# Napoliee/Expressive-FastSpeech2-Mandarin

Measured on AMD Instinct MI355X. Metric: mel-frames/sec/GPU (batch-64 synth) at 1/2/4/8 MI355X; RTF, higher is better.
Workload: dtype bf16; 1 GPU; cfg2: batch=64 x 64 phonemes per GPU, ESD-Chinese-Singing-MFA model.yaml, FastSpeech2.forward eval bf16; global_batch=64, seq_len=64, mel_frames_per_gpu_batch=24883, T_max=430, parallelism=dp1 (independent shards, no collective), hip_graph=True

## Files before the change

expressive-fastspeech2-mandarin_amd/csrc/lr.hip:

```cpp
#include <cstdlib>
#include <type_traits>

#include "fs2_common.h"
#include "fs2hip_prosody.h"

namespace {

constexpr int kScanThreads = 256;
constexpr int kLdsCum = 2048;

__device__ __forceinline__ int64_t frames_of(const void *dur, int kind, float d_control, const float *d_map,
                                             int64_t idx, float *d_rounded) {
  if (kind == FS2_DUR_I64) {
    int64_t d = reinterpret_cast<const int64_t *>(dur)[idx];
    return d > 0 ? d : 0;
  }
  float v = reinterpret_cast<const float *>(dur)[idx];
  if (kind == FS2_DUR_LOGPRED) {
    float r = rintf(expf(v) - 1.0f) * (d_map != nullptr ? d_map[idx] : d_control);
    r = r < 0.0f ? 0.0f : r;
    if (d_rounded) d_rounded[idx] = r;
    v = r;
  }
  if (!(v > 0.0f)) return 0;
  if (v >= 9.2e18f) return INT64_MAX / 4;
  return (int64_t)v;
}

__global__ __launch_bounds__(kScanThreads) void lr_durations_kernel(const void *dur, int kind, float d_control,
                                                                    const float *d_map, int L, int32_t *cum,
                                                                    int64_t *mel_len, float *d_rounded) {
  const int b = blockIdx.x;
  const int tid = threadIdx.x;
  const int lane = tid & 63, wid = tid >> 6;
  const int per = (L + kScanThreads - 1) / kScanThreads;
  const int i0 = min(tid * per, L), i1 = min(i0 + per, L);
  const int64_t base = (int64_t)b * L;
// ... 330 lines not shown
    bf16 *pb = a.proj_out + ((int64_t)cu_b + t0) * NP;
    const int lanes = 192 / cg * cg;
    if (tid < lanes) {
      const int c = (tid % cg) * 8, r1 = tid / cg, rs = lanes / cg;
      for (int r0 = r1; r0 < rows; r0 += RB * rs) {
        float4 tv[RB][2], sv[RB][2];
#pragma unroll
        for (int u = 0; u < RB; ++u) {
          const int r = min(r0 + u * rs, rows - 1);
          const int sidx = src[r];
          const float *tp = tb + (int64_t)r * NP + c;
          tv[u][0] = *reinterpret_cast<const float4 *>(tp);
          tv[u][1] = *reinterpret_cast<const float4 *>(tp + 4);
          if (sidx >= 0) {
            const float *sp = sb + (int64_t)sidx * NP + c;
            sv[u][0] = *reinterpret_cast<const float4 *>(sp);
            sv[u][1] = *reinterpret_cast<const float4 *>(sp + 4);
          } else {
            sv[u][0] = sv[u][1] = make_float4(0.f, 0.f, 0.f, 0.f);
          }
        }
#pragma unroll
        for (int u = 0; u < RB; ++u) {
          const int r = r0 + u * rs;
          if (r < rows) {
            const bf16x8 o{(bf16)(tv[u][0].x + sv[u][0].x), (bf16)(tv[u][0].y + sv[u][0].y),
                           (bf16)(tv[u][0].z + sv[u][0].z), (bf16)(tv[u][0].w + sv[u][0].w),
                           (bf16)(tv[u][1].x + sv[u][1].x), (bf16)(tv[u][1].y + sv[u][1].y),
                           (bf16)(tv[u][1].z + sv[u][1].z), (bf16)(tv[u][1].w + sv[u][1].w)};
            __builtin_nontemporal_store(o, reinterpret_cast<bf16x8 *>(pb + (int64_t)r * NP + c));
          }
        }
      }
    }
  }
}

__global__ __launch_bounds__(256) void length_mask_kernel(const int64_t *__restrict__ lens, int width, int64_t n,
                                                          bool *__restrict__ mask) {
  const int64_t i = (int64_t)blockIdx.x * 256 + threadIdx.x;
  if (i >= n) return;
  const int64_t b = i / width;
  mask[i] = (int64_t)(i - b * width) >= lens[b];
}

__global__ __launch_bounds__(256) void seq_cu_kernel(const int64_t *__restrict__ lens, int B, int T,
                                                     int32_t *__restrict__ cu) {
  __shared__ int32_t part[257];
  const int tid = threadIdx.x;
  const int per = (B + 255) / 256;
  const int i0 = min(tid * per, B), i1 = min(i0 + per, B);
  int32_t local = 0;
  for (int i = i0; i < i1; ++i) {
    const int64_t l = lens[i];
    local += (int32_t)(l < 0 ? 0 : (l > T ? T : l));
  }
  part[tid + 1] = local;
  if (tid == 0) part[0] = 0;
  __syncthreads();
  if (tid == 0)
    for (int i = 1; i <= 256; ++i) part[i] += part[i - 1];
  __syncthreads();
  int32_t run = part[tid];
  for (int i = i0; i < i1; ++i) {
    cu[i] = run;
    const int64_t l = lens[i];
// ... 445 lines not shown
  }();
  const int R = rows_env;
  const dim3 grid((unsigned)((T_out + R - 1) / R), (unsigned)B);
  auto go = [&](auto TXv, auto TOv) {
    using TX = decltype(TXv);
    using TO = decltype(TOv);
    auto launch = [&](auto RC) {
      constexpr int RR = decltype(RC)::value;
      if (a.pe != nullptr)
        hipLaunchKernelGGL((lr_fused_kernel<TX, TO, true, RR>), grid, dim3(256), 0, s, a);
      else
        hipLaunchKernelGGL((lr_fused_kernel<TX, TO, false, RR>), grid, dim3(256), 0, s, a);
    };
    if (R == 128)
      launch(std::integral_constant<int, 128>{});
    else if (R == 64)
      launch(std::integral_constant<int, 64>{});
    else
      launch(std::integral_constant<int, 32>{});
  };
  if (x_dtype == FS2_BF16 && out_dtype == FS2_BF16)
    go(bf16{}, bf16{});
  else if (x_dtype == FS2_F32 && out_dtype == FS2_F32)
    go(0.0f, 0.0f);
  else if (x_dtype == FS2_F32 && out_dtype == FS2_BF16)
    go(0.0f, bf16{});
  else if (x_dtype == FS2_BF16 && out_dtype == FS2_F32)
    go(bf16{}, 0.0f);
  else
    return FS2_EUNSUPPORTED;
  FS2_CHECK_LAUNCH();
  return FS2_OK;
}
```

expressive-fastspeech2-mandarin_amd/fs2amd/_lib.py:

```python
import ctypes
import os

import torch

HERE = os.path.dirname(os.path.abspath(__file__))
DEFAULT_LIB = os.path.join(HERE, "_lib", "libfs2hip.so")

FS2_F32, FS2_BF16, FS2_FP8 = 0, 1, 2
FS2_I16 = 3
FS2_F64 = 4
PITCH_T_MAX, PITCH_T_MAX_NOFILL, OUTLIER_LDS_BYTES = 131072, 4096, 65536
F0_GROUP, F0_LDS_BYTES = 8, 65536
RESAMPLE_LDS_BYTES = 81920
MAS_LDS_BYTES, MAS_LDS_SMALL, FORWARD_SUM_LDS_BYTES = 163840, 32768, 65536
MAS_AUTO, MAS_LDS, MAS_GLOBAL = 0, 1, 2
ALIGN_SIZE_CAP = 1 << 24
DTW_LDS_BYTES, DTW_LDS_SMALL = 163840, 32768
DTW_AUTO, DTW_LDS, DTW_GLOBAL = 0, 1, 2
EVAL_SIZE_CAP = 1 << 24
F0_TRACK_THR, F0_TRACK_CAP_MAX, F0_TRACK_BINS_MAX, F0_TRACK_STEP_MAX, F0_TRACK_TB = 100, 101, 256, 63, 64
F0_TRACK_LDS_BYTES = 65536
VAD_SUMS_BYTES, VAD_AREA_BYTES, VAD_TILE_FRAMES, VAD_CHUNK_FRAMES, VAD_B_MAX = 32768, 32768, 192, 256, 65535
PVOC_BLOCK, PVOC_J_CAP, PVOC_B_MAX = 64, 2 ** 31 - 1, 65535
IIR_BLOCK, IIR_CHUNK, IIR_S_MAX, IIR_TABLE_LEN, IIR_B_MAX, LOUD_H_MAX = 64, 16384, 8, 412, 65535, 32768
# ... 62 lines not shown
        ("residual2", _p), ("out_div", _f),
        ("group_n", _i), ("group_cin", _i),
    ]


class Ffn8Desc(ctypes.Structure):

    _fields_ = [
        ("x8", _p), ("x8_row_stride", _i64), ("res", _p), ("res_row_stride", _i64), ("w", _p),
        ("cs1", _p), ("b1", _p), ("inv_sf", _f), ("cs2", _p), ("b2", _p),
        ("B", _i), ("T", _i), ("D", _i), ("F", _i), ("KS", _i), ("pad", _i),
        ("ln_gamma", _p), ("ln_beta", _p), ("ln_eps", _f),
        ("out", _p), ("out_row_stride", _i64), ("out8", _p), ("out8_row_stride", _i64), ("out8_scale", _f),
        ("rows_dev", _p), ("row_pos", _p), ("rows_max", _i),
    ]


class WconvDesc(ctypes.Structure):

    _fields_ = [
        ("x", _p), ("x_row_stride", _i64), ("w", _p), ("bias", _p),
        ("B", _i), ("T", _i), ("Cin", _i), ("N", _i), ("KS", _i), ("pad", _i), ("epilogue", _i),
        ("out", _p), ("out_row_stride", _i64), ("w2", _p), ("bias2", _p), ("residual", _p), ("res_row_stride", _i64),
        ("rows_dev", _p), ("row_pos", _p), ("rows_max", _i),
    ]


class PnHead3Desc(ctypes.Structure):

    _fields_ = [
        ("x", _p), ("x_row_stride", _i64), ("x_rows", _i64), ("rowmap", _p), ("mel_w", _p), ("mel_b", _p),
        ("mel", _p), ("mel_row_stride", _i64), ("mel_bf16", _p), ("w", _p * 3), ("bias", _p * 3),
        ("B", _i), ("T", _i), ("out", _p), ("out_row_stride", _i64),
    ]


class CondDesc(ctypes.Structure):

    _fields_ = [
        ("speakers", _p), ("speaker_table", _p), ("n_speaker", _i), ("emotions", _p), ("emo_table", _p),
        ("n_emo", _i), ("d_emo", _i), ("arousals", _p), ("aro_table", _p), ("n_aro", _i), ("d_aro", _i),
        ("valences", _p), ("val_table", _p), ("n_val", _i), ("d_val", _i), ("lin_w", _p), ("lin_b", _p),
        ("spk_out", _p), ("emo_out", _p),
    ]


class CondGrads(ctypes.Structure):

    _fields_ = [("d_speaker_table", _p), ("d_emo_table", _p), ("d_aro_table", _p), ("d_val_table", _p),
                ("d_lin_w", _p), ("d_lin_b", _p)]


class FfnDesc(ctypes.Structure):

    _fields_ = [
        ("x", _p), ("x_row_stride", _i64),
        ("w", _p), ("b1", _p), ("b2", _p),
        ("B", _i), ("T", _i), ("D", _i), ("F", _i), ("KS", _i), ("pad", _i),
        ("ln_gamma", _p), ("ln_beta", _p), ("ln_eps", _f),
        ("lens", _p), ("addvec1", _p), ("addvec2", _p),
        ("out", _p), ("out_row_stride", _i64),
        ("rows_dev", _p), ("row_pos", _p),
        ("nsplit", _i), ("splitk_ws", _p), ("splitk_ws_bytes", _i64), ("rows_max", _i),
        ("tile_rows", _i),
        ("wqkv", _p), ("bqkv", _p), ("qkv_out", _p), ("qkv_row_stride", _i64), ("nqkv", _i),
        ("pre_att", _p), ("pre_att_row_stride", _i64), ("pre_w", _p), ("pre_b", _p), ("pre_gamma", _p),
# ... 266 lines not shown
    if bitmap == DTW_LDS and not fits:
        return FS2_EUNSUPPORTED, None
    return FS2_OK, DTW_GLOBAL if bitmap == DTW_GLOBAL or not fits else DTW_LDS


SIGNATURES_F0_TRACK = {
    "fs2_f0_track_lds_bytes": (_i64, [_i, _i]),
    "fs2_f0_track_workspace_bytes": (_i64, [_i, _i, _i, _i, _i]),
    "fs2_f0_track": (_i, [_p, _p, _i, _i, _i, _d, _i, _i, _d, _d, _p, _p, _p, _p, _p, _i, _p, _p, _i, _d, _d, _p, _i64,
                          _p, _p, _p, _p]),
}


SIGNATURES_VAD = {
    "fs2_vad_frames": (_i64, [_i64, _i64]),
    "fs2_vad_workspace_bytes": (_i64, [_i64, _i64, _i64, _i64]),
    "fs2_vad_lds_bytes": (_i64, [_i64, _i64]),
    "fs2_vad_power": (_i, [_p, _i, _i64, _p, _i, _i, _i, _i, _p, _p, _p, _i64, _p]),
    "fs2_vad_intervals": (_i, [_p, _p, _p, _i, _i, _i, _d, _d, _i, _i64, _i, _i, _p, _p, _p, _p, _p]),
    "fs2_vad_cut": (_i, [_p, _i, _i64, _p, _i, _i, _i, _p, _p, _p]),
}


SIGNATURES_PVOC = {
    "fs2_pvoc_frames": (_i64, [_i64, _d]),
    "fs2_phase_vocoder": (_i, [ctypes.POINTER(PvocDesc), _p]),
}


SIGNATURES_POSTNET = {
    "fs2_pn_head3": (_i, [ctypes.POINTER(PnHead3Desc), _p]),
}

SIGNATURES_IIR = {
    "fs2_iir_blocks": (_i64, [_i64]),
    "fs2_iir_chunks": (_i64, [_i64]),
    "fs2_loudness_blocks": (_i64, [_i64, _i64]),
    "fs2_loudness_workspace_bytes": (_i64, [_i64, _i64, _i64]),
    "fs2_sosfilt": (_i, [_p, _i, _i64, _p, _i, _i, _p, _p, _i, _p, _p, _p, _p, _p]),
    "fs2_loudness_gate": (_i, [_p, _p, _i, _i, _i, _d, _d, _p, _p, _p, _i64, _p]),
    "fs2_gain_int16": (_i, [_p, _i, _i64, _p, _i, _i, _p, _d, _d, _p, _p, _p, _p, _p, _p]),
}


def iir_blocks(n):
    return 0 if n < 1 else (n - 1) // IIR_BLOCK + 1


def iir_chunks(n):
    return 0 if n < 1 else (n - 1) // IIR_CHUNK + 1


def loudness_blocks(n, H):
    return 0 if n < 1 or n < 4 * H else (n - 4 * H) // H + 1


def loudness_workspace_bytes(B, n_max, H):
    if B < 1 or n_max < 1 or H < 1:
        return 0
    J = loudness_blocks(n_max, H)
    if J < 1:
        return 0
    return min(8 * B * ((J + 3) + J + (J + 1) // 2), (1 << 63) - 1)


def iir_status(B, n_max, S, row_stride):
# ... 102 lines not shown
        return 0
    if max(n_bins, max_step) > 1 << 24:
        return (1 << 63) - 1
    return 8 * (4 * (n_bins + 2 * max_step) + 2 * n_bins) + F0_TRACK_TB * 2 * n_bins + 8


def f0_dp_ulps(W, tau):
    return 2 * W + tau + 6


def header_symbols(header_path):
    import re

    text = open(header_path).read()
    return sorted(set(re.findall(r"\b(fs2_[a-z0-9_]+)\s*\(", text)) - {"fs2_conv_desc"})


_LIB = None
CSRC = os.path.join(os.path.dirname(HERE), "csrc")
HEADER = os.path.join(os.path.dirname(os.path.dirname(HERE)), "include", "fs2hip.h")
HEADER_PROSODY = os.path.join(os.path.dirname(HEADER), "fs2hip_prosody.h")
HEADER_AUDIO = os.path.join(os.path.dirname(HEADER), "fs2hip_audio.h")
HEADER_AUDIO_INV = os.path.join(os.path.dirname(HEADER), "fs2hip_audio_inv.h")
HEADER_PREP = os.path.join(os.path.dirname(HEADER), "fs2hip_prep.h")
HEADER_F0 = os.path.join(os.path.dirname(HEADER), "fs2hip_f0.h")
HEADER_RESAMPLE = os.path.join(os.path.dirname(HEADER), "fs2hip_resample.h")
HEADER_ALIGN = os.path.join(os.path.dirname(HEADER), "fs2hip_align.h")
HEADER_EVAL = os.path.join(os.path.dirname(HEADER), "fs2hip_eval.h")
HEADER_F0_TRACK = os.path.join(os.path.dirname(HEADER), "fs2hip_f0_track.h")
HEADER_VAD = os.path.join(os.path.dirname(HEADER), "fs2hip_vad.h")
HEADER_PVOC = os.path.join(os.path.dirname(HEADER), "fs2hip_pvoc.h")
HEADER_IIR = os.path.join(os.path.dirname(HEADER), "fs2hip_iir.h")
HEADER_POSTNET = os.path.join(os.path.dirname(HEADER), "fs2hip_postnet.h")
EXTRA_HEADERS = ("fs2hip_prosody.h", "fs2hip_audio.h", "fs2hip_audio_inv.h", "fs2hip_prep.h", "fs2hip_f0.h",
                 "fs2hip_resample.h", "fs2hip_align.h", "fs2hip_eval.h", "fs2hip_f0_track.h", "fs2hip_vad.h",
                 "fs2hip_pvoc.h", "fs2hip_iir.h", "fs2hip_postnet.h")


def source_build_id(csrc=CSRC, header=HEADER):
    import hashlib

    if not os.path.isdir(csrc) or not os.path.exists(header):
        return None
    h = hashlib.sha256()
    for name in sorted(f for f in os.listdir(csrc) if f.endswith((".hip", ".h"))):
        h.update(name.encode())
        with open(os.path.join(csrc, name), "rb") as f:
            h.update(f.read())
    with open(header, "rb") as f:
        h.update(b"fs2hip.h")
        h.update(f.read())
    for name in EXTRA_HEADERS:
        with open(os.path.join(os.path.dirname(header), name), "rb") as f:
            h.update(name.encode())
            h.update(f.read())
    return h.hexdigest()[:16]


def lib_path():
    return os.environ.get("FS2_LIB", DEFAULT_LIB)


def load():
    global _LIB
    if _LIB is not None:
        return _LIB
    path = lib_path()
    if not os.path.exists(path):
        raise RuntimeError(
            f"fs2amd: HIP library not found at {path}. Build it with `python -c 'import __graft_entry__ as g; "
            f"g.build()'` (hipcc --offload-arch=gfx950). There is no CPU fallback.")
    lib = ctypes.CDLL(path, mode=ctypes.RTLD_GLOBAL)
    allow_missing = "FS2_LIB" in os.environ and os.environ.get("FS2_LIB_ALLOW_MISSING") == "1"
    for name, (res, args) in list(SIGNATURES.items()) + list(SIGNATURES_PROSODY.items()) + \
            list(SIGNATURES_AUDIO.items()) + list(SIGNATURES_AUDIO_INV.items()) + list(SIGNATURES_PREP.items()) + \
            list(SIGNATURES_F0.items()) + list(SIGNATURES_RESAMPLE.items()) + list(SIGNATURES_ALIGN.items()) + \
            list(SIGNATURES_EVAL.items()) + list(SIGNATURES_F0_TRACK.items()) + list(SIGNATURES_VAD.items()) + \
            list(SIGNATURES_PVOC.items()) + list(SIGNATURES_IIR.items()) + list(SIGNATURES_POSTNET.items()):
        if allow_missing and not hasattr(lib, name):
            continue
        fn = getattr(lib, name)
        fn.restype = res
        fn.argtypes = args
    if "FS2_LIB" not in os.environ:
        want = source_build_id()
        got = lib.fs2_build_id().decode()
        if want is not None and got != want:
            raise RuntimeError(f"fs2amd: {path} was built from other sources (fs2_build_id {got}, sources "
                               f"{want}); rebuild with `python -c 'import __graft_entry__ as g; g.build()'`")
    _LIB = lib
    return lib


def check(rc, what):
    if rc != FS2_OK:
        msg = load().fs2_status_string(rc).decode()
        raise RuntimeError(f"{what} failed: fs2 status {rc} ({msg})")
```

expressive-fastspeech2-mandarin_amd/fs2amd/ops.py:

```python
import collections
import ctypes
import os

import torch

from . import _lib as L

_lib = L.load()


def _ptr(t):
    return None if t is None else ctypes.c_void_p(t.data_ptr())


def _stream(t):
    return ctypes.c_void_p(torch.cuda.current_stream(t.device).cuda_stream)


def _dt(t):
    if t.dtype == torch.bfloat16:
        return L.FS2_BF16
    if t.dtype == torch.float32:
        return L.FS2_F32
    if t.dtype == torch.float8_e4m3fn:
# ... 1103 lines not shown
            and ppe.shape[0] >= T_out and NP % 8 == 0 and 8 <= NP <= 1536, (tuple(psrc.shape), tuple(ppe.shape), B, Lx, T_out)
        pout = lay.empty(NP, torch.bfloat16)
    if dur is not None:
        dur = dur.contiguous()
        cum = torch.empty(B, Lx, device=dev, dtype=torch.int32)
        mel_len = torch.empty(B, device=dev, dtype=torch.int64)
        d_rounded = torch.empty(B, Lx, device=dev, dtype=torch.float32) if logpred else None
        if torch.is_tensor(d_control):
            c, dmap = control_arg(d_control, B, Lx, dev, "d_control")
            L.check(_lib.fs2_lr_fused_proj_map(_ptr(x), _dt(x), _ptr(dur), _dur_kind(dur, logpred), c, _ptr(dmap), None,
                                               None, B, Lx, D, int(T_out), _ptr(pe), _ptr(lens), _ptr(lay.cu),
                                               _ptr(lay.row_pos), _ptr(lay.rowmap), _ptr(out), od, _ptr(cum),
                                               _ptr(mel_len), _ptr(d_rounded), _ptr(psrc), _ptr(ppe), NP, _ptr(pout),
                                               _stream(x)), "fs2_lr_fused_proj_map")
            res = (out, lay, cum, mel_len, d_rounded)
            return res + (pout,) if proj is not None else res
        L.check(_lib.fs2_lr_fused_proj(_ptr(x), _dt(x), _ptr(dur), _dur_kind(dur, logpred), float(d_control), None,
                                       None, B, Lx, D, int(T_out), _ptr(pe), _ptr(lens), _ptr(lay.cu),
                                       _ptr(lay.row_pos), _ptr(lay.rowmap), _ptr(out), od, _ptr(cum), _ptr(mel_len),
                                       _ptr(d_rounded), _ptr(psrc), _ptr(ppe), NP, _ptr(pout), _stream(x)),
                "fs2_lr_fused_proj")
        res = (out, lay, cum, mel_len, d_rounded)
    else:
        if torch.is_tensor(d_control):
            raise ValueError("fs2amd.lr_fused: a d_control map needs the durations (dur=..., logpred=True)")
        L.check(_lib.fs2_lr_fused_proj(_ptr(x), _dt(x), None, 0, 1.0, _ptr(cum), _ptr(mel_len), B, Lx, D, int(T_out),
                                       _ptr(pe), _ptr(lens), _ptr(lay.cu), _ptr(lay.row_pos), _ptr(lay.rowmap),
                                       _ptr(out), od, None, None, None, _ptr(psrc), _ptr(ppe), NP, _ptr(pout),
                                       _stream(x)), "fs2_lr_fused_proj")
        res = (out, lay)
    return res + (pout,) if proj is not None else res


def length_regulate(x, duration, max_len=None, return_index_map=False, d_control=None):
    if d_control is not None:
        return _length_regulate_logpred(x, duration, max_len, return_index_map, d_control)
    if max_len:
        _gpu(x, duration)
        x, duration = x.contiguous(), duration.contiguous()
        B, Lx, D = x.shape
        T_out = int(max_len)
        cum = torch.empty(B, Lx, device=x.device, dtype=torch.int32)
        mel_len = torch.empty(B, device=x.device, dtype=torch.int64)
        out = torch.empty(B, T_out, D, device=x.device, dtype=x.dtype)
        im = torch.empty(B, T_out, device=x.device, dtype=torch.int32) if return_index_map else None
        L.check(_lib.fs2_length_regulate(_ptr(x), _dt(x), _ptr(duration), _dur_kind(duration, False), 1.0, B, Lx, D,
                                         T_out, None, _ptr(out), _dt(x), _ptr(cum), _ptr(mel_len), None, _ptr(im),
                                         _stream(x)), "fs2_length_regulate")
        return (out, mel_len, im) if return_index_map else (out, mel_len)
    cum, mel_len, _ = lr_durations(duration)
    T_out = int(mel_len.max().item()) if mel_len.numel() else 0
    res = lr_expand(x, cum, mel_len, T_out, index_map=return_index_map)
    if return_index_map:
        return res[0], mel_len, res[1]
    return res, mel_len


def _length_regulate_logpred(x, log_d, max_len, return_index_map, d_control):
    _gpu(x, log_d)
    x, log_d = x.contiguous(), log_d.contiguous()
    if log_d.dtype != torch.float32:
        raise TypeError(f"fs2amd.length_regulate: log-duration predictions must be float32, got {log_d.dtype}")
    B, Lx, D = x.shape
    if max_len:
        T_out = int(max_len)
        c, dmap = control_arg(d_control, B, Lx, x.device, "d_control")
# ... 1308 lines not shown
```

expressive-fastspeech2-mandarin_amd/fs2amd/runtime.py:

```python
import os
from types import SimpleNamespace

import numpy as np
import torch

from . import _lib as L
from . import ops
from .model import sinusoid_table


def _mask(lengths, width):
    if lengths.is_cuda:
        return ops.length_mask(lengths, width)
    ids = torch.arange(0, width, device=lengths.device).unsqueeze(0).expand(lengths.shape[0], -1)
    return ids >= lengths.unsqueeze(1).expand(-1, width)


def _pe(P, which, n):
    tab = P.enc_pe if which == "enc" else P.dec_pe
    if n <= tab.shape[0]:
        return tab
    key = f"_pe_{which}_{n}"
    if not hasattr(P, key):
        setattr(P, key, sinusoid_table(n, tab.shape[1]).to(tab.device))
    return getattr(P, key)


def _qkv_pe(P, n):
    q = P.dec_qkv_pe
    if n <= q.table.shape[0]:
        return q.table
    key = f"_qkv_pe_{n}"
    if not hasattr(P, key):
        from .packing import qkv_pe_rows
        setattr(P, key, qkv_pe_rows(_pe(P, "dec", n)[:n], q.attn, q.compute))
    return getattr(P, key)


def lr_proj_ok(P, x):
    if os.environ.get("FS2_LR_PROJ", "1") == "0" or getattr(P, "dec_qkv_pe", None) is None or CALIB is not None:
        return False
    lp = P.dec_layers[0]
    return x.dtype == torch.bfloat16 and (lp.fp8 is None or lp.fp8.wqkv is None) and lp.n_head * lp.d_k == x.shape[-1]


TIMERS = None
_STACK = ["enc"]


def _record_event():
    e = torch.cuda.Event(enable_timing=True)
    e.record()
    return e


class _Timed:

    __slots__ = ("tag", "e0")

    def __init__(self, tag):
        self.tag = tag

    def __enter__(self):
        if TIMERS is not None:
            self.e0 = _record_event()
        return self

    def __exit__(self, *exc):
        if TIMERS is not None and exc[0] is None:
            TIMERS.append((self.e0, _record_event(), self.tag))
        return False


def _tm(op):
    return _Timed(f"{_STACK[0]}:{op}")
CALIB = None
# ... 434 lines not shown
        if T_dec != T_out:
            x = x[:, :T_dec].contiguous()
    if T_dec != T_out:
        dec_lens = torch.clamp(dec_lens, max=T_dec)
    x = _stack(P, P.dec_layers, x, dec_lens, timed=True)
    if pn_head3_ok(P, x, postnet_valid):
        mel, y = _pn_head3(P, x, x.shape[0], x.shape[1])
        return mel, _postnet_convs(P, y, mel, first=3), st
    mel_bf = _mel_copy(P, x, x.shape[:2])
    mel = ops.conv1d(x, P.mel_w, P.mel_b, cin=P.d_model, ks=1, pad=0, compute=P.compute, epilogue=L.EPI_BIAS,
                     out_dtype=L.FS2_F32, out2=mel_bf)
    return mel, _postnet(P, mel, mel_bf, dec_lens if postnet_valid else None, rows_hint), st


def decode_packed(P, st, x, dec_lens, T_lay, rows_hint=None):
    x, lay, qkv0 = _lr_packed(P, st, x, dec_lens, T_lay, rows_hint)
    return _stack(P, P.dec_layers, x, None, layout=lay, timed=True, qkv0=qkv0), lay


def decode_packed_head(P, st, x, dec_lens, T_lay, rows_hint=None):
    x, lay, qkv0 = _lr_packed(P, st, x, dec_lens, T_lay, rows_hint)
    x1, qkv1 = _stack(P, P.dec_layers[:1], x, None, layout=lay, timed=True, qkv0=qkv0, tail_next=P.dec_layers[1])
    return x1, lay, qkv1


def decode_packed_rest(P, x1, lay, qkv1):
    return _stack(P, P.dec_layers[1:], x1, None, layout=lay, timed=True, qkv0=qkv1)


def _lr_packed(P, st, x, dec_lens, T_lay, rows_hint=None):
    qkv0 = None
    if lr_fused_ok(x):
        proj = None
        if lr_proj_ok(P, x):
            xw = getattr(st, "xw", None)
            if xw is None:
                xw = phoneme_qkv0(P, x)
            proj = (xw.view(-1, xw.shape[-1]), _qkv_pe(P, T_lay))
        with _Timed("va:lr"):
            if st.cum is None:
                r = ops.lr_fused(x, dec_lens, T_lay, pe=_pe(P, "dec", T_lay), out_dtype=P.act_dtype,
                                 dur=st.dur_pending, proj=proj)
                x, lay, st.cum, st.mel_len = r[:4]
            else:
                r = ops.lr_fused(x, dec_lens, T_lay, pe=_pe(P, "dec", T_lay), out_dtype=P.act_dtype,
                                 cum=st.cum, mel_len=st.mel_len, proj=proj)
                x, lay = r[:2]
            qkv0 = r[-1] if proj is not None else None
    else:
        _ensure_lr(st)
        lay = ops.SeqLayout(dec_lens, T_lay)
        x = ops.lr_expand(x, st.cum, st.mel_len, T_lay, pe=_pe(P, "dec", T_lay), out_dtype=P.act_dtype,
                          out_layout=lay)
    lay.rows_hint = None if rows_hint is None else ops.rows_bucket(rows_hint, lay.capacity)
    return x, lay, qkv0


def phoneme_qkv0(P, x):
    lp = P.dec_layers[0]
    with _Timed("dec:qkv0"):
        return ops.conv1d(x, lp.wqkv, None, cin=x.shape[-1], ks=1, pad=0, compute=P.compute, epilogue=L.EPI_BIAS,
                          out_dtype=L.FS2_F32)


def split_stage2_ok(P):
    return (os.environ.get("FS2_SYNTH_SPLIT", "0") == "1" and len(P.dec_layers) >= 2
            and all(lp.fp8 is None for lp in P.dec_layers))

# ... 272 lines not shown
```

Measured before the change: 18.93 million mel-frames/s.

## Fuse phoneme QKV projection into length-regulator entry kernel

```diff
diff --git a/expressive-fastspeech2-mandarin_amd/csrc/lr.hip b/expressive-fastspeech2-mandarin_amd/csrc/lr.hip
--- a/expressive-fastspeech2-mandarin_amd/csrc/lr.hip
+++ b/expressive-fastspeech2-mandarin_amd/csrc/lr.hip
@@ -3,6 +3,7 @@
 
 #include "fs2_common.h"
 #include "fs2hip_prosody.h"
+#include "lr_entry_sizes.h"
 
 namespace {
 
@@ -399,6 +400,235 @@
           }
         }
       }
+    }
+  }
+}
+
+struct LrEntryArgs {
+  LrFusedArgs a;
+  const bf16 *w;
+};
+
+template <bool HAS_PE>
+__global__ __launch_bounds__(256) void lr_entry_kernel(LrEntryArgs e) {
+  constexpr int PH = FS2_LR_ENTRY_PH, D = FS2_LR_ENTRY_D, NP = FS2_LR_ENTRY_NP, YS = FS2_LRE_YSTRIDE;
+  constexpr int WN = NP / 4;
+  constexpr int NB = WN / 16;
+  constexpr int PF = 4;
+  const LrFusedArgs &a = e.a;
+  const int b = blockIdx.y, jb = blockIdx.x, p0 = jb * PH;
+  const int tid = threadIdx.x, lane = tid & 63, wv = tid >> 6;
+  const int L = a.L, T = a.T;
+  __shared__ __attribute__((aligned(16))) float ylds[PH * YS];
+  __shared__ int32_t scum[kLdsCum];
+  __shared__ int src[FS2_LRE_PASS];
+  __shared__ int64_t wtot[4];
+  __shared__ int32_t wcu[4];
+  __shared__ int64_t s_ml;
+  const bool first = jb == 0;
+  auto clen = [&](int j) {
+    const int64_t l = a.lens[j];
+    return (int32_t)(l < 0 ? 0 : (l > T ? T : l));
+  };
+  int32_t part = 0;
+  for (int j = tid; j < b; j += 256) part += clen(j);
+  if (a.dur != nullptr) {
+    const int per = (L + 255) / 256;
+    const int i0 = min(tid * per, L), i1 = min(i0 + per, L);
+    const int64_t base = (int64_t)b * L;
+    int64_t local = 0;
+    for (int i = i0; i < i1; ++i) local += frames_of(a.dur, a.dur_kind, a.d_control, a.d_map, base + i, nullptr);
+    int64_t incl = local;
+#pragma unroll
+    for (int o = 1; o < 64; o <<= 1) {
+      const int64_t y = __shfl_up(incl, o, 64);
+      if (lane >= o) incl += y;
+    }
+    if (lane == 63) wtot[wv] = incl;
+    __syncthreads();
+    int64_t run = incl - local;
+    for (int w = 0; w < wv; ++w) run += wtot[w];
+    for (int i = i0; i < i1; ++i) {
+      run += frames_of(a.dur, a.dur_kind, a.d_control, a.d_map, base + i, first ? a.d_rounded : nullptr);
+      const int32_t c = (int32_t)(run < 0x7fffffff ? run : 0x7fffffff);
+      scum[i] = c;
+      if (first) a.cum[base + i] = c;
+    }
+    if (tid == 0) {
+      const int64_t total = (wtot[0] + wtot[1]) + (wtot[2] + wtot[3]);
+      s_ml = total;
+      if (first) a.mel_len[b] = total;
+    }
+  } else {
+    const int32_t *c = a.cum_in + (int64_t)b * L;
+    for (int i = tid; i < L; i += 256) scum[i] = c[i];
+    if (tid == 0) s_ml = a.mel_len_in[b];
+  }
+#pragma unroll
+  for (int o = 32; o > 0; o >>= 1) part += __shfl_xor(part, o, 64);
+  if (lane == 0) wcu[wv] = part;
+  __syncthreads();
+  const int32_t cu_b = (wcu[0] + wcu[1]) + (wcu[2] + wcu[3]);
+  const int32_t len_b = clen(b);
+  if (first && tid == 0) {
+    a.cu[b] = cu_b;
+    if (b == a.B - 1) a.cu[a.B] = cu_b + len_b;
+  }
+
+  const int64_t ml = s_ml;
+  const int lim = (int)(ml < 0 ? 0 : (ml < (int64_t)T ? ml : (int64_t)T));
+  int fr[3];
+  lre_range(scum, L, jb, lim, T, fr);
+  const int f0 = fr[0], f1 = fr[1], fe = fr[2];
+  if (fe <= f0) return;
+  const int rend = min(T, (int)len_b);
+  const bool need_y = f0 < min(f1, rend);
+  const int pl = min(p0 + PH - 1, L - 1);
+
+  const bf16 *xb = reinterpret_cast<const bf16 *>(a.x) + (int64_t)b * L * D;
+  bf16x8 xf[8], wf[PF][8];
+  auto wload = [&](int nb, bf16x8(&dst)[8]) {
+    const int g = wv * NB + nb;
+    const bf16 *wp = e.w + ((int64_t)(g >> 2) * (D / 32) * 4 + (g & 3)) * 512 + lane * 8;
+#pragma unroll
+    for (int s = 0; s < 8; ++s) dst[s] = *reinterpret_cast<const bf16x8 *>(wp + s * 4 * 512);
+  };
+  if (need_y) {
+#pragma unroll
+    for (int k = 0; k < PF - 1; ++k) wload(k, wf[k]);
+    const bf16 *xr = xb + (int64_t)min(p0 + (lane & 15), pl) * D + 8 * (lane >> 4);
+#pragma unroll
+    for (int s = 0; s < 8; ++s) xf[s] = *reinterpret_cast<const bf16x8 *>(xr + 32 * s);
+  }
+
+  auto sources = [&](int c0, int n) {
+    for (int i = tid; i < n; i += 256) {
+      const int t = c0 + i;
+      src[i] = t < f1 ? lre_src(scum, L, jb, t) - p0 : -1;
+      if (a.rowmap != nullptr) a.rowmap[(int64_t)b * T + t] = t < len_b ? cu_b + t : -1;
+      if (a.row_pos != nullptr && t < len_b) a.row_pos[cu_b + t] = make_int2(t, len_b);
+    }
+  };
+  auto gather = [&](int c0, int n) {
+    constexpr int U = 8, vpr = D >> 3;
+    const int rows = min(n, rend - c0);
+    if (rows <= 0) return;
+    const int total = rows * vpr;
+    bf16 *ob = reinterpret_cast<bf16 *>(a.out) + ((int64_t)cu_b + c0) * D;
+    for (int base = tid; base < total; base += 256 * U) {
+      float v[U][8];
+#pragma unroll
+      for (int u = 0; u < U; ++u) {
+        const int ee = base + u * 256;
+        const int r = ee / vpr;
+        const int col = (ee - r * vpr) << 3;
+        const int sidx = ee < total ? src[r] : -1;
+        if (sidx >= 0) {
+          load8(xb + (int64_t)(p0 + sidx) * D + col, v[u]);
+        } else {
+#pragma unroll
+          for (int q = 0; q < 8; ++q) v[u][q] = 0.0f;
+        }
+        if constexpr (HAS_PE) {
+          if (ee < total) {
+            float pv[8];
+            load8(a.pe + (int64_t)(c0 + r) * D + col, pv);
+#pragma unroll
+            for (int q = 0; q < 8; ++q) v[u][q] += pv[q];
+          }
+        }
+      }
+#pragma unroll
+      for (int u = 0; u < U; ++u) {
+        const int ee = base + u * 256;
+        if (ee < total) {
+          bf16x8 o;
+#pragma unroll
+          for (int q = 0; q < 8; ++q) o[q] = (bf16)v[u][q];
+          bf16x8 *dst = reinterpret_cast<bf16x8 *>(ob + (int64_t)ee * 8);
+          if (a.store == 0)
+            __builtin_nontemporal_store(o, dst);
+          else if (a.store == 1)
+            *dst = o;
+          else
+            __builtin_amdgcn_raw_buffer_store_b128(__builtin_bit_cast(__attribute__((ext_vector_type(4))) unsigned, o),
+                                                   __builtin_amdgcn_make_buffer_rsrc(dst, (short)0, 16, 0x00020000), 0u,
+                                                   0, 16);
+        }
+      }
+    }
+  };
+  auto project = [&]() {
+#pragma unroll
+    for (int nb = 0; nb < NB; ++nb) {
+      if (nb + PF - 1 < NB) wload(nb + PF - 1, wf[(nb + PF - 1) % PF]);
+      f32x4 acc = {0.f, 0.f, 0.f, 0.f};
+#pragma unroll
+      for (int s = 0; s < 8; ++s) acc = __builtin_amdgcn_mfma_f32_16x16x32_bf16(wf[nb % PF][s], xf[s], acc, 0, 0, 0);
+      *reinterpret_cast<float4 *>(&ylds[(lane & 15) * YS + wv * WN + nb * 16 + 4 * (lane >> 4)]) =
+          make_float4(acc[0] + 0.0f, acc[1] + 0.0f, acc[2] + 0.0f, acc[3] + 0.0f);
+    }
+  };
+  constexpr int EU = 8, CG = NP >> 3;
+  float4 tv[EU][2];
+  int off[EU], yo[EU];
+  auto ex_load = [&](int c0, int total, int base) {
+    const float *tb = a.proj_pe + (int64_t)c0 * NP;
+#pragma unroll
+    for (int u = 0; u < EU; ++u) {
+      const int ee = min(base + u * 256, total - 1);
+      const int r = ee / CG;
+      const int c = (ee - r * CG) << 3;
+      const int sidx = src[r];
+      off[u] = r * NP + c;
+      yo[u] = sidx >= 0 ? sidx * YS + c : -1;
+      tv[u][0] = *reinterpret_cast<const float4 *>(tb + off[u]);
+      tv[u][1] = *reinterpret_cast<const float4 *>(tb + off[u] + 4);
+    }
+  };
+  auto ex_store = [&](int c0, int total, int base) {
+    bf16 *pb = a.proj_out + ((int64_t)cu_b + c0) * NP;
+#pragma unroll
+    for (int u = 0; u < EU; ++u) {
+      if (base + u * 256 < total) {
+        float4 s0 = make_float4(0.f, 0.f, 0.f, 0.f), s1 = s0;
+        if (yo[u] >= 0) {
+          s0 = *reinterpret_cast<const float4 *>(&ylds[yo[u]]);
+          s1 = *reinterpret_cast<const float4 *>(&ylds[yo[u] + 4]);
+        }
+        const bf16x8 o{(bf16)(tv[u][0].x + s0.x), (bf16)(tv[u][0].y + s0.y), (bf16)(tv[u][0].z + s0.z),
+                       (bf16)(tv[u][0].w + s0.w), (bf16)(tv[u][1].x + s1.x), (bf16)(tv[u][1].y + s1.y),
+                       (bf16)(tv[u][1].z + s1.z), (bf16)(tv[u][1].w + s1.w)};
+        __builtin_nontemporal_store(o, reinterpret_cast<bf16x8 *>(pb + off[u]));
+      }
+    }
+  };
+
+  int n = min(FS2_LRE_PASS, fe - f0);
+  sources(f0, n);
+  __syncthreads();
+  gather(f0, n);
+  int total = max(min(n, rend - f0), 0) * CG;
+  if (total > 0) ex_load(f0, total, tid);
+  if (need_y) project();
+  __syncthreads();
+  if (total > 0) {
+    ex_store(f0, total, tid);
+    for (int base = tid + 256 * EU; base < total; base += 256 * EU) {
+      ex_load(f0, total, base);
+      ex_store(f0, total, base);
+    }
+  }
+  for (int c0 = f0 + FS2_LRE_PASS; c0 < fe; c0 += FS2_LRE_PASS) {
+    __syncthreads();
+    n = min(FS2_LRE_PASS, fe - c0);
+    sources(c0, n);
+    __syncthreads();
+    gather(c0, n);
+    total = max(min(n, rend - c0), 0) * CG;
+    for (int base = tid; base < total; base += 256 * EU) {
+      ex_load(c0, total, base);
+      ex_store(c0, total, base);
     }
   }
 }
@@ -910,3 +1140,80 @@
   FS2_CHECK_LAUNCH();
   return FS2_OK;
 }
+
+extern "C" int64_t fs2_lr_entry_workgroups(int64_t B, int64_t L) { return lre_workgroups(B, L); }
+
+extern "C" int fs2_lr_entry_plan(const int32_t *cum, int L, int64_t mel_len, int T, int32_t *src) {
+  if (cum == nullptr || src == nullptr || L < 1 || T < 0) return FS2_EINVAL;
+  const int lim = (int)(mel_len < 0 ? 0 : (mel_len < (int64_t)T ? mel_len : (int64_t)T));
+  for (int t = 0; t < T; ++t) src[t] = -2;
+  for (int j = 0; j < (int)lre_blocks(L); ++j) {
+    int r[3];
+    lre_range(cum, L, j, lim, T, r);
+    for (int t = r[0]; t < r[2]; ++t) {
+      if (src[t] != -2) return FS2_EINVAL;
+      src[t] = t < r[1] ? lre_src(cum, L, j, t) : -1;
+    }
+  }
+  return FS2_OK;
+}
+
+extern "C" int fs2_lr_entry(const fs2_lr_entry_desc *d, fs2_stream_t stream) {
+  if (d == nullptr) return FS2_EINVAL;
+  if (d->x == nullptr || d->out == nullptr || d->layout_lens == nullptr || d->cu == nullptr || d->w == nullptr ||
+      d->proj_pe == nullptr || d->proj_out == nullptr)
+    return FS2_EINVAL;
+  if (d->d_map != nullptr && (d->dur == nullptr || d->dur_kind != FS2_DUR_LOGPRED)) return FS2_EINVAL;
+  if (d->dur != nullptr) {
+    if (d->cum == nullptr || d->mel_len == nullptr || d->dur_kind < FS2_DUR_I64 || d->dur_kind > FS2_DUR_LOGPRED)
+      return FS2_EINVAL;
+    if (d->dur_kind == FS2_DUR_LOGPRED && d->d_rounded == nullptr) return FS2_EINVAL;
+  } else if (d->cum_in == nullptr || d->mel_len_in == nullptr) {
+    return FS2_EINVAL;
+  }
+  const int rc = lre_check(d->B, d->L, d->D, d->NP, d->T, d->x_dtype, d->out_dtype);
+  if (rc != FS2_OK) return rc;
+  if (d->B == 0) return FS2_OK;
+  if (d->T == 0)
+    return fs2_lr_fused_proj_map(d->x, d->x_dtype, d->dur, d->dur_kind, d->d_control, d->d_map, d->cum_in, d->mel_len_in,
+                                 d->B, d->L, d->D, 0, d->pe, d->layout_lens, d->cu, d->row_pos, d->rowmap, d->out,
+                                 d->out_dtype, d->cum, d->mel_len, d->d_rounded, nullptr, nullptr, 0, nullptr, stream);
+  LrEntryArgs e{};
+  LrFusedArgs &a = e.a;
+  a.x = d->x;
+  a.dur = d->dur;
+  a.dur_kind = d->dur_kind;
+  a.d_control = d->d_control;
+  a.d_map = d->d_map;
+  a.cum_in = d->cum_in;
+  a.mel_len_in = d->mel_len_in;
+  a.lens = d->layout_lens;
+  a.B = d->B;
+  a.L = d->L;
+  a.D = d->D;
+  a.T = d->T;
+  a.pe = d->pe;
+  a.out = d->out;
+  a.cum = d->cum;
+  a.mel_len = d->mel_len;
+  a.d_rounded = d->d_rounded;
+  a.cu = d->cu;
+  a.row_pos = reinterpret_cast<int2 *>(d->row_pos);
+  a.rowmap = d->rowmap;
+  static const int store_env = [] {
+    const char *s = getenv("FS2_LR_STORE");
+    return s == nullptr ? 0 : (s[0] == 'p' ? 1 : s[0] == 's' ? 2 : 0);
+  }();
+  a.store = store_env;
+  a.proj_pe = d->proj_pe;
+  a.NP = d->NP;
+  a.proj_out = reinterpret_cast<bf16 *>(d->proj_out);
+  e.w = reinterpret_cast<const bf16 *>(d->w);
+  const dim3 grid((unsigned)lre_blocks(d->L), (unsigned)d->B);
+  if (d->pe != nullptr)
+    hipLaunchKernelGGL(lr_entry_kernel<true>, grid, dim3(256), 0, as_stream(stream), e);
+  else
+    hipLaunchKernelGGL(lr_entry_kernel<false>, grid, dim3(256), 0, as_stream(stream), e);
+  FS2_CHECK_LAUNCH();
+  return FS2_OK;
+}
diff --git a/expressive-fastspeech2-mandarin_amd/csrc/lr_entry_sizes.h b/expressive-fastspeech2-mandarin_amd/csrc/lr_entry_sizes.h
--- /dev/null
+++ b/expressive-fastspeech2-mandarin_amd/csrc/lr_entry_sizes.h
@@ -0,0 +1,66 @@
+#pragma once
+#include <stdint.h>
+
+#include "fs2hip_lr_entry.h"
+
+#ifdef __HIPCC__
+#define FS2_LRE_HD __host__ __device__
+#else
+#define FS2_LRE_HD
+#endif
+
+#define FS2_LRE_YSTRIDE 772
+#define FS2_LRE_PASS 512
+#define FS2_LRE_B_MAX 4096
+
+FS2_LRE_HD static inline int64_t lre_blocks(int64_t L) { return L < 1 ? 0 : (L + FS2_LR_ENTRY_PH - 1) / FS2_LR_ENTRY_PH; }
+
+FS2_LRE_HD static inline int64_t lre_workgroups(int64_t B, int64_t L) { return B < 1 ? 0 : B * lre_blocks(L); }
+
+FS2_LRE_HD static inline int64_t lre_lds_bytes(void) {
+  return (int64_t)FS2_LR_ENTRY_PH * FS2_LRE_YSTRIDE * 4 + (int64_t)FS2_LR_ENTRY_L_MAX * 4 + FS2_LRE_PASS * 4 + 4 * 8 +
+         4 * 4 + 8;
+}
+
+FS2_LRE_HD static inline int64_t lre_max_bytes(int64_t B, int64_t L, int64_t T) {
+  const int64_t rows = B * T;
+  int64_t m = rows * FS2_LR_ENTRY_NP * 2;
+  const int64_t xb = B * L * FS2_LR_ENTRY_D * 2, tb = T * FS2_LR_ENTRY_NP * 4;
+  if (xb > m) m = xb;
+  if (tb > m) m = tb;
+  return m;
+}
+
+FS2_LRE_HD static inline int lre_check(int64_t B, int64_t L, int64_t D, int64_t NP, int64_t T, int x_dtype,
+                                       int out_dtype) {
+  if (B < 0 || L < 1 || D < 1 || NP < 1 || T < 0) return FS2_EINVAL;
+  if (x_dtype != FS2_BF16 || out_dtype != FS2_BF16) return FS2_EUNSUPPORTED;
+  if (D != FS2_LR_ENTRY_D || NP != FS2_LR_ENTRY_NP) return FS2_EUNSUPPORTED;
+  if (L > FS2_LR_ENTRY_L_MAX || B > FS2_LRE_B_MAX) return FS2_EUNSUPPORTED;
+  if (T > INT32_MAX || lre_max_bytes(B, L, T) >= ((int64_t)1 << 31)) return FS2_EUNSUPPORTED;
+  return FS2_OK;
+}
+
+FS2_LRE_HD static inline void lre_range(const int32_t *cum, int L, int j, int lim, int T, int r[3]) {
+  const int p0 = j * FS2_LR_ENTRY_PH;
+  const int pl = p0 + FS2_LR_ENTRY_PH - 1 < L - 1 ? p0 + FS2_LR_ENTRY_PH - 1 : L - 1;
+  const bool last = pl == L - 1;
+  const int c0 = p0 > 0 ? cum[p0 - 1] : 0;
+  r[0] = c0 < lim ? c0 : lim;
+  if (r[0] < 0) r[0] = 0;
+  r[1] = last ? lim : (cum[pl] < lim ? cum[pl] : lim);
+  if (r[1] < r[0]) r[1] = r[0];
+  r[2] = last ? (T > r[1] ? T : r[1]) : r[1];
+}
+
+FS2_LRE_HD static inline int lre_src(const int32_t *cum, int L, int j, int t) {
+  const int p0 = j * FS2_LR_ENTRY_PH;
+  const int pl = p0 + FS2_LR_ENTRY_PH - 1 < L - 1 ? p0 + FS2_LR_ENTRY_PH - 1 : L - 1;
+  int s = pl;
+#pragma unroll
+  for (int q = FS2_LR_ENTRY_PH - 1; q >= 0; --q) {
+    const int i = p0 + q;
+    if (i <= pl && cum[i] > t) s = i;
+  }
+  return s;
+}
diff --git a/expressive-fastspeech2-mandarin_amd/fs2amd/_lib.py b/expressive-fastspeech2-mandarin_amd/fs2amd/_lib.py
--- a/expressive-fastspeech2-mandarin_amd/fs2amd/_lib.py
+++ b/expressive-fastspeech2-mandarin_amd/fs2amd/_lib.py
@@ -118,6 +118,16 @@
         ("x", _p), ("x_row_stride", _i64), ("x_rows", _i64), ("rowmap", _p), ("mel_w", _p), ("mel_b", _p),
         ("mel", _p), ("mel_row_stride", _i64), ("mel_bf16", _p), ("w", _p * 3), ("bias", _p * 3),
         ("B", _i), ("T", _i), ("out", _p), ("out_row_stride", _i64),
+    ]
+
+
+class LrEntryDesc(ctypes.Structure):
+
+    _fields_ = [
+        ("x", _p), ("x_dtype", _i), ("dur", _p), ("dur_kind", _i), ("d_control", _f), ("d_map", _p),
+        ("cum_in", _p), ("mel_len_in", _p), ("layout_lens", _p), ("B", _i), ("L", _i), ("D", _i), ("T", _i),
+        ("pe", _p), ("w", _p), ("proj_pe", _p), ("NP", _i), ("out", _p), ("out_dtype", _i), ("proj_out", _p),
+        ("cum", _p), ("mel_len", _p), ("d_rounded", _p), ("cu", _p), ("row_pos", _p), ("rowmap", _p),
     ]
 
 
@@ -450,6 +460,30 @@
     "fs2_pn_head3": (_i, [ctypes.POINTER(PnHead3Desc), _p]),
 }
 
+SIGNATURES_LR_ENTRY = {
+    "fs2_lr_entry": (_i, [ctypes.POINTER(LrEntryDesc), _p]),
+    "fs2_lr_entry_workgroups": (_i64, [_i64, _i64]),
+    "fs2_lr_entry_plan": (_i, [_p, _i, _i64, _i, _p]),
+}
+LR_ENTRY_PH = 16
+LR_ENTRY_L_MAX = 2048
+LR_ENTRY_B_MAX = 4096
+
+
+def lr_entry_workgroups(B, L):
+    return 0 if B < 1 or L < 1 else B * ((L + LR_ENTRY_PH - 1) // LR_ENTRY_PH)
+
+
+def lr_entry_status(B, L, D, NP, T, x_dtype=1, out_dtype=1):
+    if B < 0 or L < 1 or D < 1 or NP < 1 or T < 0:
+        return FS2_EINVAL
+    if x_dtype != 1 or out_dtype != 1 or D != 256 or NP != 768 or L > LR_ENTRY_L_MAX or B > LR_ENTRY_B_MAX:
+        return FS2_EUNSUPPORTED
+    if T > 2 ** 31 - 1 or max(B * T * NP * 2, B * L * D * 2, T * NP * 4) >= 2 ** 31:
+        return FS2_EUNSUPPORTED
+    return FS2_OK
+
+
 SIGNATURES_IIR = {
     "fs2_iir_blocks": (_i64, [_i64]),
     "fs2_iir_chunks": (_i64, [_i64]),
@@ -618,9 +652,10 @@
 HEADER_PVOC = os.path.join(os.path.dirname(HEADER), "fs2hip_pvoc.h")
 HEADER_IIR = os.path.join(os.path.dirname(HEADER), "fs2hip_iir.h")
 HEADER_POSTNET = os.path.join(os.path.dirname(HEADER), "fs2hip_postnet.h")
+HEADER_LR_ENTRY = os.path.join(os.path.dirname(HEADER), "fs2hip_lr_entry.h")
 EXTRA_HEADERS = ("fs2hip_prosody.h", "fs2hip_audio.h", "fs2hip_audio_inv.h", "fs2hip_prep.h", "fs2hip_f0.h",
                  "fs2hip_resample.h", "fs2hip_align.h", "fs2hip_eval.h", "fs2hip_f0_track.h", "fs2hip_vad.h",
-                 "fs2hip_pvoc.h", "fs2hip_iir.h", "fs2hip_postnet.h")
+                 "fs2hip_pvoc.h", "fs2hip_iir.h", "fs2hip_postnet.h", "fs2hip_lr_entry.h")
 
 
 def source_build_id(csrc=CSRC, header=HEADER):
@@ -662,7 +697,8 @@
             list(SIGNATURES_AUDIO.items()) + list(SIGNATURES_AUDIO_INV.items()) + list(SIGNATURES_PREP.items()) + \
             list(SIGNATURES_F0.items()) + list(SIGNATURES_RESAMPLE.items()) + list(SIGNATURES_ALIGN.items()) + \
             list(SIGNATURES_EVAL.items()) + list(SIGNATURES_F0_TRACK.items()) + list(SIGNATURES_VAD.items()) + \
-            list(SIGNATURES_PVOC.items()) + list(SIGNATURES_IIR.items()) + list(SIGNATURES_POSTNET.items()):
+            list(SIGNATURES_PVOC.items()) + list(SIGNATURES_IIR.items()) + list(SIGNATURES_POSTNET.items()) + \
+            list(SIGNATURES_LR_ENTRY.items()):
         if allow_missing and not hasattr(lib, name):
             continue
         fn = getattr(lib, name)
diff --git a/expressive-fastspeech2-mandarin_amd/fs2amd/ops.py b/expressive-fastspeech2-mandarin_amd/fs2amd/ops.py
--- a/expressive-fastspeech2-mandarin_amd/fs2amd/ops.py
+++ b/expressive-fastspeech2-mandarin_amd/fs2amd/ops.py
@@ -1159,6 +1159,52 @@
     return res + (pout,) if proj is not None else res
 
 
+def lr_entry(x, lens, T_out, w, proj_pe, pe=None, dur=None, logpred=False, d_control=1.0, cum=None, mel_len=None):
+    _gpu(x, lens, pe, dur, cum, mel_len, w, proj_pe)
+    if x.dtype != torch.bfloat16 or w.dtype != torch.bfloat16 or proj_pe.dtype != torch.float32:
+        raise TypeError("fs2amd.lr_entry: bf16 rows and weights, an f32 position table")
+    x = x.contiguous()
+    B, Lx, D = x.shape
+    dev = x.device
+    NP = proj_pe.shape[-1]
+    if w.numel() != NP * D or not w.is_contiguous() or proj_pe.dim() != 2 or not proj_pe.is_contiguous() \
+            or proj_pe.shape[0] < T_out or (pe is not None and (pe.dtype != torch.float32 or not pe.is_contiguous()
+                                                                 or pe.shape[0] < T_out or pe.shape[1] != D)):
+        raise ValueError(f"fs2amd.lr_entry: w {tuple(w.shape)}, proj_pe {tuple(proj_pe.shape)} for x {tuple(x.shape)}, "
+                         f"T_out {T_out}")
+    lens = lens.to(torch.int64).contiguous()
+    lay = SeqLayout.deferred(B, T_out, dev)
+    out = lay.empty(D, torch.bfloat16)
+    pout = lay.empty(NP, torch.bfloat16)
+    d = L.LrEntryDesc()
+    d.x, d.x_dtype, d.B, d.L, d.D, d.T = _ptr(x), L.FS2_BF16, B, Lx, D, int(T_out)
+    d.layout_lens, d.pe, d.w, d.proj_pe, d.NP = _ptr(lens), _ptr(pe), _ptr(w), _ptr(proj_pe), NP
+    d.out, d.out_dtype, d.proj_out = _ptr(out), L.FS2_BF16, _ptr(pout)
+    d.cu, d.row_pos, d.rowmap = _ptr(lay.cu), _ptr(lay.row_pos), _ptr(lay.rowmap)
+    d.d_control = 1.0
+    if dur is not None:
+        dur = dur.contiguous()
+        cum = torch.empty(B, Lx, device=dev, dtype=torch.int32)
+        mel_len = torch.empty(B, device=dev, dtype=torch.int64)
+        d_rounded = torch.empty(B, Lx, device=dev, dtype=torch.float32) if logpred else None
+        dmap = None
+        if torch.is_tensor(d_control):
+            c, dmap = control_arg(d_control, B, Lx, dev, "d_control")
+        else:
+            c = float(d_control)
+        d.dur, d.dur_kind, d.d_control, d.d_map = _ptr(dur), _dur_kind(dur, logpred), c, _ptr(dmap)
+        d.cum, d.mel_len, d.d_rounded = _ptr(cum), _ptr(mel_len), _ptr(d_rounded)
+        res = (out, lay, cum, mel_len, d_rounded, pout)
+    else:
+        if torch.is_tensor(d_control):
+            raise ValueError("fs2amd.lr_entry: a d_control map needs the durations (dur=..., logpred=True)")
+        cum, mel_len = cum.contiguous(), mel_len.contiguous()
+        d.cum_in, d.mel_len_in = _ptr(cum), _ptr(mel_len)
+        res = (out, lay, pout)
+    L.check(_lib.fs2_lr_entry(ctypes.byref(d), _stream(x)), "fs2_lr_entry")
+    return res
+
+
 def length_regulate(x, duration, max_len=None, return_index_map=False, d_control=None):
     if d_control is not None:
         return _length_regulate_logpred(x, duration, max_len, return_index_map, d_control)
diff --git a/expressive-fastspeech2-mandarin_amd/fs2amd/runtime.py b/expressive-fastspeech2-mandarin_amd/fs2amd/runtime.py
--- a/expressive-fastspeech2-mandarin_amd/fs2amd/runtime.py
+++ b/expressive-fastspeech2-mandarin_amd/fs2amd/runtime.py
@@ -42,6 +42,21 @@
         return False
     lp = P.dec_layers[0]
     return x.dtype == torch.bfloat16 and (lp.fp8 is None or lp.fp8.wqkv is None) and lp.n_head * lp.d_k == x.shape[-1]
+
+
+LR_ENTRY_MAX_WG = 512
+
+
+def lr_entry_on():
+    return os.environ.get("FS2_LR_ENTRY", "1") != "0"
+
+
+def lr_entry_ok(P, x):
+    from . import _lib
+    B, Lx, D = x.shape
+    return (lr_entry_on() and lr_proj_ok(P, x) and D == 256 and P.dec_qkv_pe.table.shape[-1] == 768
+            and getattr(P.dec_layers[0], "wqf", None) is not None and Lx <= _lib.LR_ENTRY_L_MAX
+            and 0 < _lib.lr_entry_workgroups(B, Lx) <= LR_ENTRY_MAX_WG)
 
 
 TIMERS = None
@@ -542,8 +557,18 @@
     qkv0 = None
     if lr_fused_ok(x):
         proj = None
+        xw = getattr(st, "xw", None)
+        if xw is None and lr_entry_ok(P, x):
+            kw = dict(dur=st.dur_pending) if st.cum is None else dict(cum=st.cum, mel_len=st.mel_len)
+            with _Timed("va:lr"):
+                r = ops.lr_entry(x, dec_lens, T_lay, P.dec_layers[0].wqf, _qkv_pe(P, T_lay), pe=_pe(P, "dec", T_lay),
+                                 **kw)
+            if st.cum is None:
+                st.cum, st.mel_len = r[2:4]
+            x, lay, qkv0 = r[0], r[1], r[-1]
+            lay.rows_hint = None if rows_hint is None else ops.rows_bucket(rows_hint, lay.capacity)
+            return x, lay, qkv0
         if lr_proj_ok(P, x):
-            xw = getattr(st, "xw", None)
             if xw is None:
                 xw = phoneme_qkv0(P, x)
             proj = (xw.view(-1, xw.shape[-1]), _qkv_pe(P, T_lay))
diff --git a/include/fs2hip_lr_entry.h b/include/fs2hip_lr_entry.h
--- /dev/null
+++ b/include/fs2hip_lr_entry.h
@@ -0,0 +1,51 @@
+#ifndef FS2HIP_LR_ENTRY_H
+#define FS2HIP_LR_ENTRY_H
+
+#include "fs2hip.h"
+
+#ifdef __cplusplus
+extern "C" {
+#endif
+
+#define FS2_LR_ENTRY_PH 16
+#define FS2_LR_ENTRY_D 256
+#define FS2_LR_ENTRY_NP 768
+#define FS2_LR_ENTRY_L_MAX 2048
+
+typedef struct fs2_lr_entry_desc {
+  const void *x;
+  int x_dtype;
+  const void *dur;
+  int dur_kind;
+  float d_control;
+  const float *d_map;
+  const int32_t *cum_in;
+  const int64_t *mel_len_in;
+  const int64_t *layout_lens;
+  int B, L, D, T;
+  const float *pe;
+  const void *w;
+  const float *proj_pe;
+  int NP;
+  void *out;
+  int out_dtype;
+  void *proj_out;
+  int32_t *cum;
+  int64_t *mel_len;
+  float *d_rounded;
+  int32_t *cu;
+  int32_t *row_pos;
+  int32_t *rowmap;
+} fs2_lr_entry_desc;
+
+int fs2_lr_entry(const fs2_lr_entry_desc *d, fs2_stream_t stream);
+
+int64_t fs2_lr_entry_workgroups(int64_t B, int64_t L);
+
+int fs2_lr_entry_plan(const int32_t *cum, int L, int64_t mel_len, int T, int32_t *src);
+
+#ifdef __cplusplus
+}
+#endif
+
+#endif
```

After: 18.72 million mel-frames/s. 0.989x the previous value.
